# davidalvarezdlt/master_thesis

Measured on NVIDIA B200. Metric: aligned_frames_per_sec, higher is better.
Workload: dtype f32

## Files before the change

### include/mt_b200.h

```cpp
#ifndef MT_B200_H
#define MT_B200_H

#include <stdint.h>

#ifdef __cplusplus
extern "C" {
#endif

#define MT_OK 0
#define MT_ERR_INVALID (-1)
#define MT_ERR_CUDA (-2)
#define MT_ERR_NO_DEVICE (-3)

typedef void *mt_stream_t;

#define MT_API __attribute__((visibility("default")))

#define MT_ALIGN_CORNERS 1
#define MT_VIS_BILINEAR 2
#define MT_GRID_AFFINE 4
#define MT_VIS_FROM_MASK 8

#define MT_REDUCE_MEAN 0
#define MT_REDUCE_SUM 1

MT_API int mt_version(void);
MT_API const char *mt_last_error(void);
MT_API int mt_set_tuning(const char *name, int value);
MT_API int mt_device_info(int *sm_count, int *cc_major, int *cc_minor);
MT_API int64_t mt_workspace_bytes(void);

MT_API int mt_warp_fwd(const float *x, int64_t x_sb, int64_t x_sc, int64_t x_sf,
                const float *vis, int64_t vis_sb, int64_t vis_sf,
                const float *grid, const float *m_target, int64_t mt_sb,
                float *x_aligned, int64_t xa_sb, int64_t xa_sc, int64_t xa_sf,
                float *v_aligned, float *v_map,
                int B, int C, int F, int H, int W, int flags, mt_stream_t stream);

MT_API int mt_warp_pack_fwd(const float *x, int64_t x_sb, int64_t x_sc, int64_t x_sf,
                     const float *vis, int64_t vis_sb, int64_t vis_sf,
                     const float *grid, const float *m_target, int64_t mt_sb,
                     const float *x_t, int64_t xt_sb, int64_t xt_sc, const float *v_t, int64_t vt_sb,
                     float *nn_in,
                     float *x_aligned, int64_t xa_sb, int64_t xa_sc, int64_t xa_sf,
                     float *v_aligned, float *v_map,
                     int B, int F, int H, int W, int flags, mt_stream_t stream);

MT_API int mt_warp_lowres_fwd(const float *x, int64_t x_sb, int64_t x_sc, int64_t x_sf,
                       const float *vis, int64_t vis_sb, int64_t vis_sf,
                       const float *flow, int gh, int gw, const float *m_target, int64_t mt_sb,
                       float *x_aligned, int64_t xa_sb, int64_t xa_sc, int64_t xa_sf,
                       float *v_aligned, float *v_map,
                       int B, int F, int H, int W, int flags, mt_stream_t stream);
MT_API int mt_warp_pack_lowres_fwd(const float *x, int64_t x_sb, int64_t x_sc, int64_t x_sf,
                            const float *vis, int64_t vis_sb, int64_t vis_sf,
                            const float *flow, int gh, int gw, const float *m_target, int64_t mt_sb,
                            const float *x_t, int64_t xt_sb, int64_t xt_sc, const float *v_t, int64_t vt_sb,
                            float *nn_in,
                            float *x_aligned, int64_t xa_sb, int64_t xa_sc, int64_t xa_sf,
                            float *v_aligned, float *v_map,
                            int B, int F, int H, int W, int flags, mt_stream_t stream);

MT_API int mt_warp_bwd_grid(const float *x, int64_t x_sb, int64_t x_sc, int64_t x_sf,
                     const float *grid,
                     const float *gout, int64_t g_sb, int64_t g_sc, int64_t g_sf,
                     float *ggrid, int B, int C, int F, int H, int W, int flags,
                     mt_stream_t stream);

MT_API int mt_warp_l1_fwd(const float *x, int64_t x_sb, int64_t x_sc, int64_t x_sf,
                   const float *vis, int64_t vis_sb, int64_t vis_sf,
                   const float *flow,
                   const float *x_target, int64_t xt_sb, int64_t xt_sc,
                   const float *v_target, int64_t vt_sb,
                   float *x_aligned, float *v_aligned, float *out3, void *workspace,
                   int B, int F, int H, int W, float weight, int flags, mt_stream_t stream);

MT_API int mt_warp_l1_bwd(const float *x, int64_t x_sb, int64_t x_sc, int64_t x_sf,
                   const float *flow,
                   const float *x_target, int64_t xt_sb, int64_t xt_sc,
                   const float *v_target, int64_t vt_sb,
                   const float *out3, const float *grad_out, float *gflow,
                   int B, int F, int H, int W, float weight, int flags, mt_stream_t stream);

MT_API int mt_mask_out(const float *flow, int64_t n, float *out, mt_stream_t stream);

MT_API int mt_masked_l1_fwd(const float *y_hat, int64_t a_sb, int64_t a_sc, int64_t a_sf,
                     const float *y, int64_t b_sb, int64_t b_sc, int64_t b_sf,
                     const float *mask, int64_t m_sb, int64_t m_sc, int64_t m_sf,
                     const uint8_t *batch_mask, float *out3, void *workspace,
                     int B, int C, int F, int64_t P, int mask_c, int64_t mask_repeat, int reduction,
                     float weight, mt_stream_t stream);
MT_API int mt_masked_l1_bwd(const float *y_hat, int64_t a_sb, int64_t a_sc, int64_t a_sf,
                     const float *y, int64_t b_sb, int64_t b_sc, int64_t b_sf,
                     const float *mask, int64_t m_sb, int64_t m_sc, int64_t m_sf,
                     const uint8_t *batch_mask, const float *out3, const float *grad_out,
                     float *grad_y_hat, float *grad_y,
                     int B, int C, int F, int64_t P, int mask_c, int reduction, float weight,
                     mt_stream_t stream);

MT_API int mt_chn_l1x3_fwd(const float *y_hat, int64_t yh_sb, int64_t yh_sc, int64_t yh_sf,
                    const float *y_comp, int64_t yc_sb, int64_t yc_sc, int64_t yc_sf,
                    const float *y_target, int64_t yt_sb, int64_t yt_sc,
                    const float *v_target, int64_t vt_sb,
                    const float *v_map, int64_t vm_sb, int64_t vm_sf,
                    float *out9, void *workspace, int B, int F, int64_t P,
                    float w_nh, float w_vh, float w_nvh, mt_stream_t stream);
MT_API int mt_chn_l1x3_bwd(const float *y_hat, int64_t yh_sb, int64_t yh_sc, int64_t yh_sf,
                    const float *y_comp, int64_t yc_sb, int64_t yc_sc, int64_t yc_sf,
                    const float *y_target, int64_t yt_sb, int64_t yt_sc,
                    const float *v_target, int64_t vt_sb,
                    const float *v_map, int64_t vm_sb, int64_t vm_sf,
                    const float *out9, const float *grad_out3, float *grad_y_hat, float *grad_y_comp,
                    int B, int F, int64_t P, float w_nh, float w_vh, float w_nvh, mt_stream_t stream);

MT_API int mt_chn_fill_step(const float *nn_out, const float *x_t, int64_t xt_sb, int64_t xt_sc,
                     const float *v_t, int64_t vt_sb, const float *m_t, int64_t mt_sb,
                     const float *v_map0, int64_t vm_sb, float *y_comp0, float *m_new, float *x_new,
                     float *inp_per, void *workspace, int B, int64_t P, mt_stream_t stream);

MT_API int mt_chn_fill_step_gated(const float *nn_out, const float *x_t, int64_t xt_sb, int64_t xt_sc,
                           const float *v_t, int64_t vt_sb, const float *m_t, int64_t mt_sb,
                           const float *v_map0, int64_t vm_sb, const float *y_prev,
                           const float *gate_per, float gate_e,
                           float *y_comp0, float *m_new, float *x_new,
                           float *inp_per, void *workspace, int B, int64_t P, mt_stream_t stream);

MT_API int mt_corr4d_fwd(const float *feats_t, const float *v_t, const float *feats_r, const float *v_r,
                  float *out, void *workspace, int64_t workspace_bytes,
                  int B, int C, int F, int P, mt_stream_t stream);
MT_API int64_t mt_corr4d_workspace_bytes(int B, int C, int F, int P);
MT_API int mt_corr4d_uses_tensor_cores(int C, int P);

MT_API int mt_corr4d_vgg_fwd(const float *feats_t, int64_t ft_sb, int64_t ft_sc,
                      const float *m_target, int64_t mt_sb,
                      const float *feats_r, int64_t fr_sb, int64_t fr_sc, int64_t fr_sf,
                      const float *m_refs, int64_t mr_sb, int64_t mr_sf, int MH, int MW,
                      float *out, int B, int C, int F, int h, int w, mt_stream_t stream);

MT_API int mt_corr4d_vgg_l1_fwd(const float *feats_t, int64_t ft_sb, int64_t ft_sc,
                         const float *m_target, int64_t mt_sb,
                         const float *feats_r, int64_t fr_sb, int64_t fr_sc, int64_t fr_sf,
                         const float *m_refs, int64_t mr_sb, int64_t mr_sf, int MH, int MW,
                         const float *pred, float *loss, void *sign, void *workspace, int64_t workspace_bytes,
                         int B, int C, int F, int h, int w, mt_stream_t stream);
MT_API int64_t mt_corr4d_l1_workspace_bytes(void);
MT_API int mt_corr4d_l1_bwd(const void *sign, const float *grad_loss, float *g_pred, int64_t n, mt_stream_t stream);

MT_API int mt_cm_match_fwd(const float *c_feats, const float *v_t, const float *v_aligned,
                    float *out, float *c_mask, void *workspace,
                    int B, int C, int f, int h, int w, int H, int W, mt_stream_t stream);
MT_API int64_t mt_cm_workspace_bytes(int B, int C, int f, int h, int w);
MT_API const float *mt_cm_workspace_gs(const void *workspace, int B, int C, int f, int h, int w);

MT_API int mt_chn_pack(const float *x_t, int64_t xt_sb, int64_t xt_sc, const float *v_t, int64_t vt_sb,
                const float *x_al, int64_t xa_sb, int64_t xa_sc, int64_t xa_sf,
                const float *v_al, int64_t va_sb, int64_t va_sf,
                const float *v_map, int64_t vm_sb, int64_t vm_sf,
                float *nn_in, int B, int F, int64_t P, mt_stream_t stream);
MT_API int mt_chn_composite_fwd(const float *nn_out, const float *x_t, int64_t xt_sb, int64_t xt_sc,
                         const float *v_t, int64_t vt_sb, float *y_hat, float *y_comp,
                         int B, int F, int64_t P, mt_stream_t stream);
MT_API int mt_chn_composite_bwd(const float *nn_out, const float *v_t, int64_t vt_sb,
                         const float *g_yhat, int64_t gy_sb, int64_t gy_sc, int64_t gy_sf,
                         const float *g_comp, int64_t gc_sb, int64_t gc_sc, int64_t gc_sf,
                         float *g_nn, int B, int F, int64_t P, mt_stream_t stream);
MT_API int mt_hole_update(const float *m_t, int64_t mt_sb, const float *v_map0, int64_t vm_sb,
                   const float *y_comp0, int64_t yc_sb, int64_t yc_sc,
                   float *m_new, float *x_new, float *inp_per, void *workspace,
                   int B, int64_t P, mt_stream_t stream);
MT_API int mt_trivial_copy(const float *x_t, int64_t xt_sb, int64_t xt_sc,
                    const float *x_al, int64_t xa_sb, int64_t xa_sc, int64_t xa_sf,
                    const float *v_map, int64_t vm_sb, int64_t vm_sf,
                    float *y, int B, int F, int64_t P, mt_stream_t stream);

MT_API int mt_flow_pack(const float *x_refs, int64_t xr_sb, int64_t xr_sc, int64_t xr_sf,
                 const float *x_t, int64_t xt_sb, int64_t xt_sc,
                 const float *m_refs, int64_t mr_sb, int64_t mr_sf, const float *m_t, int64_t mt_sb,
                 const float *flow, int64_t fl_sb, int64_t fl_sf, int64_t fl_sy, int64_t fl_sx, int64_t fl_sc,
                 float *nn_in, int B, int F, int H, int W, mt_stream_t stream);

MT_API int mt_cpn_align_host(const float *x_refs, const float *m_refs, const float *m_target,
                      const float *theta, float *x_aligned, float *v_aligned, float *v_maps,
                      int B, int F, int H, int W);
MT_API int mt_dfpn_align_host(const float *x_refs, const float *m_refs, const float *m_target,
                       const float *flow, float *x_aligned, float *v_aligned, float *v_maps,
                       int B, int F, int H, int W);

#ifdef __cplusplus
}
#endif
#endif
```

### master_thesis_b200/csrc/warp.cu

```cuda
#include <math.h>

#include "mt_common.cuh"
#include "warp_common.cuh"

namespace mt {
namespace {

constexpr int kCols = 128;
#ifndef MT_WARP_ROWS
#define MT_WARP_ROWS 2
#endif
#ifndef MT_TAP_REUSE
#define MT_TAP_REUSE 1
#endif
constexpr int kRows = MT_WARP_ROWS;
constexpr bool kTapReuse = MT_TAP_REUSE != 0;
constexpr int kIters = 1;
#ifndef MT_WARP_MINB
#define MT_WARP_MINB 8
#endif
#ifndef MT_WARP_MINB1
#define MT_WARP_MINB1 10
#endif
#ifndef MT_WARP_MINB4
#define MT_WARP_MINB4 4
#endif
#ifndef MT_WARPB_MINB
#define MT_WARPB_MINB 6
#endif
#ifndef MT_WARPL1F_MINB
#define MT_WARPL1F_MINB 8
#endif
#ifndef MT_WARPL1B_MINB
#define MT_WARPL1B_MINB 8
#endif

struct WarpFwdArgs {
    const float *x, *vis, *grid, *m_target;
    float *x_al, *v_al, *v_map;
    int x_sb, x_sc, x_sf, vis_sb, vis_sf, mt_sb, xa_sb, xa_sc, xa_sf;
    int F, P;
    int iters;
    unsigned f_magic;
    Sampler sp;
    bool from_mask;
    const float *x_t, *v_t;
    float *nn_in;
    int xt_sb, xt_sc, vt_sb;
    int gh, gw;
    float gsy, gsx;
    int early_trigger;
};
constexpr int kMaxRowsPerCta = 32;

template <int C, int U, int VIS, bool AFFINE, bool FULL, bool PACK = false, bool LOWRES = false>
__global__ void __launch_bounds__(kCols, U >= 4 ? MT_WARP_MINB4 : (U == 1 ? MT_WARP_MINB1 : MT_WARP_MINB)) warp_fwd_kernel(const WarpFwdArgs a) {
    static_assert(!(AFFINE && LOWRES), "a theta needs no resize");
    pdl_wait();
    if (a.early_trigger) pdl_launch();
    __shared__ float s_by[kMaxRowsPerCta];
    __shared__ Lin s_ly[LOWRES ? kMaxRowsPerCta : 1];
    const int W = a.sp.W, H = a.sp.H;
    const bool live = (int)(blockIdx.x * kCols + threadIdx.x) < W;
    const int x = min((int)(blockIdx.x * kCols + threadIdx.x), W - 1);
    const int rows_cta = U * a.iters;
    const int yb = blockIdx.y * rows_cta;
    const unsigned n = blockIdx.z;
    const int b = a.f_magic ? (int)__umulhi(n, a.f_magic) : (int)n, f = (int)n - b * a.F;
    const bool ac = a.sp.ac;
    if (AFFINE) {
        if ((int)threadIdx.x < rows_cta)
            s_by[threadIdx.x] = base_coord(min(yb + (int)threadIdx.x, H - 1), H, a.sp.stepy, ac);
        __syncthreads();
    }
    Lin lx;
    if (LOWRES) {
        if ((int)threadIdx.x < rows_cta) s_ly[threadIdx.x] = lin_index(min(yb + (int)threadIdx.x, H - 1), a.gh, H, a.gsy);
        lx = lin_index(x, a.gw, W, a.gsx);
        __syncthreads();
    }
    const int xo = b * a.x_sb + f * a.x_sf;
    const float *__restrict__ vp = a.vis + (b * a.vis_sb + f * a.vis_sf);
    const int xao = b * a.xa_sb + f * a.xa_sf;
    const int mto = b * a.mt_sb;

    float t1 = 0.f, t2 = 0.f, t4 = 0.f, t5 = 0.f, bxt0 = 0.f, bxt3 = 0.f;
    if (AFFINE) {
        const float *th = a.grid + n * 6;
        const float bx = base_coord(x, W, a.sp.stepx, ac);
        bxt0 = __fmul_rn(bx, __ldg(th));
        bxt3 = __fmul_rn(bx, __ldg(th + 3));
        t1 = __ldg(th + 1); t2 = __ldg(th + 2); t4 = __ldg(th + 4); t5 = __ldg(th + 5);
    }
    const float wm2 = a.sp.wmax - 1.0f, hm2 = a.sp.hmax - 1.0f;

    constexpr bool kDense = !AFFINE && !LOWRES;
    float2 g_next[U];
    if (kDense) {
#pragma unroll
        for (int k = 0; k < U; ++k)
            g_next[k] = (yb + k < H) ? __ldcs(reinterpret_cast<const float2 *>(a.grid) + ((int)n * a.P + (yb + k) * W + x))
                                     : make_float2(0.0f, 0.0f);
    }
#pragma unroll 1
    for (int it = 0; it < a.iters; ++it) {
        const int y0 = yb + it * U;
        if (y0 >= H) break;
        const int p0 = y0 * W + x;
        const int np0 = (int)n * a.P + p0;
        float mtv[U];
        if (FULL || PACK || a.v_map) {
#pragma unroll
            for (int k = 0; k < U; ++k) mtv[k] = (y0 + k < H) ? __ldcs(a.m_target + (mto + p0 + k * W)) : 0.0f;
        }
        float xtv[PACK ? 3 : 1][U], vtv[U];
        if (PACK) {
#pragma unroll
            for (int k = 0; k < U; ++k) {
                const bool in = y0 + k < H;
                vtv[k] = in ? __ldg(a.v_t + (b * a.vt_sb + p0 + k * W)) : 0.0f;
#pragma unroll
                for (int c = 0; c < 3; ++c) xtv[c][k] = in ? __ldg(a.x_t + (b * a.xt_sb + c * a.xt_sc + p0 + k * W)) : 0.0f;
            }
        }
        float ix[U], iy[U], xw[U], yn[U];
        float wnw[U], wne[U], wsw[U], wse[U];
        bool interior = true;
#pragma unroll
        for (int k = 0; k < U; ++k) {
            float gx, gy;
            if (AFFINE) {
                const float by = s_by[it * U + k];
                gx = __fadd_rn(__fmaf_rn(by, t1, bxt0), t2);
                gy = __fadd_rn(__fmaf_rn(by, t4, bxt3), t5);
            } else if (LOWRES) {
                const Lin ly = s_ly[it * U + k];
                const float2 *fl = reinterpret_cast<const float2 *>(a.grid) + (int)n * (a.gh * a.gw);
                const float2 g = lin_flow(fl + ly.i0 * a.gw, fl + ly.i1 * a.gw, lx, ly.l0, ly.l1);
                gx = g.x; gy = g.y;
            } else {
                gx = g_next[k].x; gy = g_next[k].y;
            }
            ix[k] = unnormalize(gx, a.sp.sfx, ac);
            iy[k] = unnormalize(gy, a.sp.sfy, ac);
            xw[k] = floorf(ix[k]);
            yn[k] = floorf(iy[k]);
            const float w = __fsub_rn(ix[k], xw[k]), e = __fsub_rn(1.0f, w);
            const float nn = __fsub_rn(iy[k], yn[k]), ss = __fsub_rn(1.0f, nn);
            wnw[k] = __fmul_rn(ss, e); wne[k] = __fmul_rn(ss, w);
            wsw[k] = __fmul_rn(nn, e); wse[k] = __fmul_rn(nn, w);
            interior = interior && (xw[k] >= 0.0f) && (xw[k] <= wm2) && (yn[k] >= 0.0f) && (yn[k] <= hm2);
        }
        if (kDense && it + 1 < a.iters) {
#pragma unroll
            for (int k = 0; k < U; ++k)
                g_next[k] = (y0 + U + k < H) ? __ldcs(reinterpret_cast<const float2 *>(a.grid) + (np0 + (U + k) * W))
                                             : make_float2(0.0f, 0.0f);
        }
        float xa[C][U], va[U];
        if (__all_sync(0xffffffffu, interior)) {
            float c00[C + 1][U], c01[C + 1][U], c10[C + 1][U], c11[C + 1][U];
            int o[U];
            bool same[U];
#pragma unroll
            for (int k = 0; k < U; ++k) {
                o[k] = (int)yn[k] * W + (int)xw[k];
                same[k] = kTapReuse && k > 0 && o[k] == o[k - 1] + W;
            }
#pragma unroll
            for (int k = 0; k < U; ++k) {
#pragma unroll
                for (int c = 0; c < C; ++c) {
                    const float *r0 = a.x + (xo + c * a.x_sc + o[k]);
                    const float *r1 = a.x + (xo + c * a.x_sc + o[k] + W);
                    c00[c][k] = 0.0f; c01[c][k] = 0.0f;
                    if (!same[k]) { c00[c][k] = __ldg(r0); c01[c][k] = __ldg(r0 + 1); }
                    c10[c][k] = __ldg(r1); c11[c][k] = __ldg(r1 + 1);
                }
                if (VIS == 2) {
                    const float *r0 = vp + o[k];
                    const float *r1 = vp + (o[k] + W);
                    c00[C][k] = 0.0f; c01[C][k] = 0.0f;
                    if (!same[k]) { c00[C][k] = __ldg(r0); c01[C][k] = __ldg(r0 + 1); }
                    c10[C][k] = __ldg(r1); c11[C][k] = __ldg(r1 + 1);
                } else {
                    c00[C][k] = __ldg(vp + ((int)rintf(iy[k]) * W + (int)rintf(ix[k])));
                }
            }
#pragma unroll
            for (int k = 1; k < U; ++k) {
#pragma unroll
                for (int c = 0; c < (VIS == 2 ? C + 1 : C); ++c) {
                    c00[c][k] = same[k] ? c10[c][k - 1] : c00[c][k];
                    c01[c][k] = same[k] ? c11[c][k - 1] : c01[c][k];
                }
            }
#pragma unroll
            for (int k = 0; k < U; ++k) {
#pragma unroll
                for (int c = 0; c < C; ++c)
                    xa[c][k] = __fmaf_rn(c11[c][k], wse[k], __fmaf_rn(c10[c][k], wsw[k],
                               __fmaf_rn(c01[c][k], wne[k], __fmul_rn(c00[c][k], wnw[k]))));
                if (VIS == 2) {
                    float v00 = c00[C][k], v01 = c01[C][k], v10 = c10[C][k], v11 = c11[C][k];
                    if (a.from_mask) {
                        v00 = __fsub_rn(1.0f, v00); v01 = __fsub_rn(1.0f, v01);
                        v10 = __fsub_rn(1.0f, v10); v11 = __fsub_rn(1.0f, v11);
                    }
                    const float vs = __fmaf_rn(v11, wse[k], __fmaf_rn(v10, wsw[k],
                                     __fmaf_rn(v01, wne[k], __fmul_rn(v00, wnw[k]))));
                    va[k] = vs > 0.5f ? 1.0f : 0.0f;
                } else {
                    va[k] = a.from_mask ? __fsub_rn(1.0f, c00[C][k]) : c00[C][k];
                }
            }
        } else {
#pragma unroll
            for (int k = 0; k < U; ++k) {
                const Bil bl = bil_params(ix[k], iy[k], a.sp);
#pragma unroll
                for (int c = 0; c < C; ++c) xa[c][k] = interp(gather(a.x + (xo + c * a.x_sc), bl, W), bl);
                if (VIS == 2) {
                    Corners cv = gather(vp, bl, W);
                    if (a.from_mask) {
                        cv.nw = (bl.y0 && bl.x0) ? __fsub_rn(1.0f, cv.nw) : 0.0f;
                        cv.ne = (bl.y0 && bl.x1) ? __fsub_rn(1.0f, cv.ne) : 0.0f;
                        cv.sw = (bl.y1 && bl.x0) ? __fsub_rn(1.0f, cv.sw) : 0.0f;
                        cv.se = (bl.y1 && bl.x1) ? __fsub_rn(1.0f, cv.se) : 0.0f;
                    }
                    va[k] = interp(cv, bl) > 0.5f ? 1.0f : 0.0f;
                } else {
                    va[k] = nearest(vp, ix[k], iy[k], a.sp, a.from_mask);
                }
            }
        }
        if (live) {
#pragma unroll
            for (int k = 0; k < U; ++k) {
                if (y0 + k >= H) break;
                if (FULL || a.x_al) {
#pragma unroll
                    for (int c = 0; c < C; ++c) st_stream1(a.x_al + (xao + p0 + c * a.xa_sc + k * W), xa[c][k]);
                }
                if (FULL || a.v_al) st_stream1(a.v_al + (np0 + k * W), va[k]);
                const float vmap = (FULL || PACK || a.v_map) ? clamp01(__fsub_rn(va[k], __fsub_rn(1.0f, mtv[k]))) : 0.0f;
                if (FULL || a.v_map)
                    st_stream1(a.v_map + (np0 + k * W), vmap);
                if (PACK) {
                    float *o = a.nn_in + ((int)n * 9 * a.P + p0 + k * W);
#pragma unroll
                    for (int c = 0; c < 3; ++c) {
                        const float m = chan_mean(c), sd = chan_std(c);
                        st_stream1(o + c * a.P, __fdiv_rn(__fsub_rn(xtv[c][k], m), sd));
                        st_stream1(o + (3 + c) * a.P, __fdiv_rn(__fsub_rn(xa[c][k], m), sd));
                    }
                    st_stream1(o + 6 * a.P, vtv[k]);
                    st_stream1(o + 7 * a.P, va[k]);
                    st_stream1(o + 8 * a.P, vmap);
                }
            }
        }
    }
}

template <int U>
struct Taps {
    float gx[U], gy[U], ix[U], iy[U], xw[U], yn[U], w[U], e[U], n[U], s[U];
    bool interior;
};

template <int U>
__device__ __forceinline__ void dense_flow_load(const float *__restrict__ flow, int np0, int y0, const Sampler &sp,
                                                float2 (&g)[U]) {
#pragma unroll
    for (int k = 0; k < U; ++k)
        g[k] = (y0 + k < sp.H) ? __ldcs(reinterpret_cast<const float2 *>(flow) + (np0 + k * sp.W)) : make_float2(0.0f, 0.0f);
}

template <int U>
__device__ __forceinline__ void dense_taps_from(const float2 (&g)[U], const Sampler &sp, Taps<U> &t) {
    const float wm2 = sp.wmax - 1.0f, hm2 = sp.hmax - 1.0f;
    t.interior = true;
#pragma unroll
    for (int k = 0; k < U; ++k) {
        t.gx[k] = g[k].x; t.gy[k] = g[k].y;
        t.ix[k] = unnormalize(t.gx[k], sp.sfx, sp.ac);
        t.iy[k] = unnormalize(t.gy[k], sp.sfy, sp.ac);
        t.xw[k] = floorf(t.ix[k]);
        t.yn[k] = floorf(t.iy[k]);
        t.w[k] = __fsub_rn(t.ix[k], t.xw[k]); t.e[k] = __fsub_rn(1.0f, t.w[k]);
        t.n[k] = __fsub_rn(t.iy[k], t.yn[k]); t.s[k] = __fsub_rn(1.0f, t.n[k]);
        t.interior = t.interior && (t.xw[k] >= 0.0f) && (t.xw[k] <= wm2) && (t.yn[k] >= 0.0f) && (t.yn[k] <= hm2);
    }
}

template <int U>
__device__ __forceinline__ void dense_taps(const float *__restrict__ flow, int np0, int y0, const Sampler &sp,
                                           Taps<U> &t) {
    float2 g[U];
    dense_flow_load<U>(flow, np0, y0, sp, g);
    dense_taps_from<U>(g, sp, t);
}

template <int C, int U>
__device__ __forceinline__ void gather_taps(const float *__restrict__ x, int xo, int x_sc, const Sampler &sp,
                                            const Taps<U> &t, Corners (&q)[C][U]) {
    if (__all_sync(0xffffffffu, t.interior)) {
#pragma unroll
        int o[U];
        bool same[U];
#pragma unroll
        for (int k = 0; k < U; ++k) {
            o[k] = (int)t.yn[k] * sp.W + (int)t.xw[k];
            same[k] = kTapReuse && k > 0 && o[k] == o[k - 1] + sp.W;
        }
#pragma unroll
        for (int k = 0; k < U; ++k) {
#pragma unroll
            for (int c = 0; c < C; ++c) {
                const float *r0 = x + (xo + c * x_sc + o[k]);
                const float *r1 = x + (xo + c * x_sc + o[k] + sp.W);
                q[c][k].nw = 0.0f; q[c][k].ne = 0.0f;
                if (!same[k]) { q[c][k].nw = __ldg(r0); q[c][k].ne = __ldg(r0 + 1); }
                q[c][k].sw = __ldg(r1); q[c][k].se = __ldg(r1 + 1);
            }
        }
#pragma unroll
        for (int k = 1; k < U; ++k) {
#pragma unroll
            for (int c = 0; c < C; ++c) {
                q[c][k].nw = same[k] ? q[c][k - 1].sw : q[c][k].nw;
                q[c][k].ne = same[k] ? q[c][k - 1].se : q[c][k].ne;
            }
        }
    } else {
#pragma unroll
        for (int k = 0; k < U; ++k) {
            const Bil bl = bil_params(t.ix[k], t.iy[k], sp);
#pragma unroll
            for (int c = 0; c < C; ++c) q[c][k] = gather(x + (xo + c * x_sc), bl, sp.W);
        }
    }
}

template <int U>
__device__ __forceinline__ float interp_k(const Corners &q, const Taps<U> &t, int k) {
    return __fmaf_rn(q.se, __fmul_rn(t.n[k], t.w[k]), __fmaf_rn(q.sw, __fmul_rn(t.n[k], t.e[k]),
           __fmaf_rn(q.ne, __fmul_rn(t.s[k], t.w[k]), __fmul_rn(q.nw, __fmul_rn(t.s[k], t.e[k])))));
}

#ifndef MT_WARPB_ROWS
#define MT_WARPB_ROWS 2
#endif
constexpr int kRowsB = MT_WARPB_ROWS;

struct WarpBwdArgs {
    const float *x, *grid, *gout;
    float *ggrid;
    int x_sb, x_sc, x_sf, g_sb, g_sc, g_sf;
    int F, P;
    unsigned f_magic;
    Sampler sp;
};

template <int C, int U>
__global__ void __launch_bounds__(kCols, MT_WARPB_MINB) warp_bwd_grid_kernel(const WarpBwdArgs a) {
    pdl_sync();
    const int W = a.sp.W, H = a.sp.H;
    const bool live = (int)(blockIdx.x * kCols + threadIdx.x) < W;
    const int x = min((int)(blockIdx.x * kCols + threadIdx.x), W - 1);
    const int y0 = blockIdx.y * U;
    const unsigned n = blockIdx.z;
    const int b = a.f_magic ? (int)__umulhi(n, a.f_magic) : (int)n, f = (int)n - b * a.F;
    const int p0 = y0 * W + x, np0 = (int)n * a.P + p0;
    const int go0 = b * a.g_sb + f * a.g_sf + p0;
    float go[C][U];
#pragma unroll
    for (int c = 0; c < C; ++c)
#pragma unroll
        for (int k = 0; k < U; ++k) go[c][k] = (y0 + k < H) ? __ldcs(a.gout + (go0 + c * a.g_sc + k * W)) : 0.0f;
    Taps<U> t;
    dense_taps<U>(a.grid, np0, y0, a.sp, t);
    Corners q[C][U];
    gather_taps<C, U>(a.x, b * a.x_sb + f * a.x_sf, a.x_sc, a.sp, t, q);
    if (!live) return;
#pragma unroll
    for (int k = 0; k < U; ++k) {
        if (y0 + k >= H) break;
        float ax = 0.0f, ay = 0.0f;
#pragma unroll
        for (int c = 0; c < C; ++c) {
            ax += ((q[c][k].ne - q[c][k].nw) * t.s[k] + (q[c][k].se - q[c][k].sw) * t.n[k]) * go[c][k];
            ay += ((q[c][k].sw - q[c][k].nw) * t.e[k] + (q[c][k].se - q[c][k].ne) * t.w[k]) * go[c][k];
        }
        __stcs(reinterpret_cast<float2 *>(a.ggrid) + (np0 + k * W), make_float2(ax * a.sp.sfx, ay * a.sp.sfy));
    }
}

struct WarpL1Args {
    const float *x, *vis, *flow, *xt, *vt;
    float *x_al, *v_al;
    float *out3; void *ws;
    const float *out3_in, *grad_out; float *gflow;
    int x_sb, x_sc, x_sf, vis_sb, vis_sf, xt_sb, xt_sc, vt_sb;
    int F, P, row_blocks;
    unsigned f_magic;
    float weight;
    Sampler sp;
    bool from_mask;
};

__device__ __forceinline__ float mask_out_of(float gx, float gy) {
    return (gx < -1.0f || gx > 1.0f || gy < -1.0f || gy > 1.0f) ? 1.0f : 0.0f;
}

template <int U, bool MAT>
__global__ void __launch_bounds__(kCols, MAT ? MT_WARPB_MINB : MT_WARPL1F_MINB) warp_l1_fwd_kernel(const WarpL1Args a) {
    pdl_sync();
    __shared__ float red[2 * 32];
    float acc[2] = {0.0f, 0.0f};
    const int W = a.sp.W, H = a.sp.H;
    const bool live = (int)(blockIdx.x * kCols + threadIdx.x) < W;
    const int x = min((int)(blockIdx.x * kCols + threadIdx.x), W - 1);
    const unsigned n = blockIdx.z;
    const int b = a.f_magic ? (int)__umulhi(n, a.f_magic) : (int)n, f = (int)n - b * a.F;
    const int xo = b * a.x_sb + f * a.x_sf;
    const int per = (a.row_blocks + (int)gridDim.y - 1) / (int)gridDim.y;
    const int rb0 = (int)blockIdx.y * per, rb1 = min(rb0 + per, a.row_blocks);
    float2 g_next[U];
    if (rb0 < rb1)
        dense_flow_load<U>(a.flow, (int)n * a.P + rb0 * U * W + x, rb0 * U, a.sp, g_next);
    for (int rb = rb0; rb < rb1; ++rb) {
        const int y0 = rb * U;
        const int p0 = y0 * W + x, np0 = (int)n * a.P + p0;
        float xt[3][U], vt[U];
#pragma unroll
        for (int k = 0; k < U; ++k) {
            const bool in = y0 + k < H;
            vt[k] = in ? __ldg(a.vt + (b * a.vt_sb + p0 + k * W)) : 0.0f;
#pragma unroll
            for (int c = 0; c < 3; ++c) xt[c][k] = in ? __ldg(a.xt + (b * a.xt_sb + c * a.xt_sc + p0 + k * W)) : 0.0f;
        }
        Taps<U> t;
        dense_taps_from<U>(g_next, a.sp, t);
        {
            const int rn = rb + 1;
            if (rn < rb1) dense_flow_load<U>(a.flow, (int)n * a.P + rn * U * W + x, rn * U, a.sp, g_next);
        }
        Corners q[3][U];
        gather_taps<3, U>(a.x, xo, a.x_sc, a.sp, t, q);
#pragma unroll
        for (int k = 0; k < U; ++k) {
            if (y0 + k >= H || !live) continue;
            const float M = __fmul_rn(vt[k], __fsub_rn(1.0f, mask_out_of(t.gx[k], t.gy[k])));
            acc[1] += M;
#pragma unroll
            for (int c = 0; c < 3; ++c) {
                const float r = interp_k<U>(q[c][k], t, k);
                acc[0] += fabsf(__fsub_rn(__fmul_rn(xt[c][k], M), __fmul_rn(r, M)));
                if (MAT && a.x_al) st_stream1(a.x_al + (((int)n * 3 + c) * a.P + p0 + k * W), r);
            }
            if (MAT && a.v_al)
                st_stream1(a.v_al + (np0 + k * W),
                           nearest(a.vis + (b * a.vis_sb + f * a.vis_sf), t.ix[k], t.iy[k], a.sp, a.from_mask));
        }
    }
    float *out3 = a.out3;
    const float weight = a.weight;
    grid_reduce_finish<2>(acc, a.ws, red, [out3, weight](const double *tot) {
        const float num = (float)tot[0], den = (float)tot[1];
        out3[0] = weight * num / (den + 1e-9f);
        out3[1] = num;
        out3[2] = den;
    });
}

template <int U>
__global__ void __launch_bounds__(kCols, MT_WARPL1B_MINB) warp_l1_bwd_kernel(const WarpL1Args a) {
    pdl_sync();
    const int W = a.sp.W, H = a.sp.H;
    const bool live = (int)(blockIdx.x * kCols + threadIdx.x) < W;
    const int x = min((int)(blockIdx.x * kCols + threadIdx.x), W - 1);
    const int y0 = blockIdx.y * U;
    const unsigned n = blockIdx.z;
    const int b = a.f_magic ? (int)__umulhi(n, a.f_magic) : (int)n, f = (int)n - b * a.F;
    const int p0 = y0 * W + x, np0 = (int)n * a.P + p0;
    const float scale = a.weight * __ldg(a.grad_out) / (__ldg(a.out3_in + 2) + 1e-9f);
    float xt[3][U], vt[U];
#pragma unroll
    for (int k = 0; k < U; ++k) {
        const bool in = y0 + k < H;
        vt[k] = in ? __ldg(a.vt + (b * a.vt_sb + p0 + k * W)) : 0.0f;
#pragma unroll
        for (int c = 0; c < 3; ++c) xt[c][k] = in ? __ldg(a.xt + (b * a.xt_sb + c * a.xt_sc + p0 + k * W)) : 0.0f;
    }
    Taps<U> t;
    dense_taps<U>(a.flow, np0, y0, a.sp, t);
    Corners q[3][U];
    gather_taps<3, U>(a.x, b * a.x_sb + f * a.x_sf, a.x_sc, a.sp, t, q);
    if (!live) return;
#pragma unroll
    for (int k = 0; k < U; ++k) {
        if (y0 + k >= H) break;
        const float M = __fmul_rn(vt[k], __fsub_rn(1.0f, mask_out_of(t.gx[k], t.gy[k])));
        float ax = 0.0f, ay = 0.0f;
#pragma unroll
        for (int c = 0; c < 3; ++c) {
            const float d = __fsub_rn(__fmul_rn(xt[c][k], M), __fmul_rn(interp_k<U>(q[c][k], t, k), M));
            const float sg = (d > 0.0f) ? 1.0f : ((d < 0.0f) ? -1.0f : 0.0f);
            const float go = -sg * M * scale;
            ax += ((q[c][k].ne - q[c][k].nw) * t.s[k] + (q[c][k].se - q[c][k].sw) * t.n[k]) * go;
            ay += ((q[c][k].sw - q[c][k].nw) * t.e[k] + (q[c][k].se - q[c][k].ne) * t.w[k]) * go;
        }
        __stcs(reinterpret_cast<float2 *>(a.gflow) + (np0 + k * W), make_float2(ax * a.sp.sfx, ay * a.sp.sfy));
    }
}

__global__ void __launch_bounds__(256) mask_out_kernel(const float *__restrict__ flow, int64_t n,
                                                       float *__restrict__ out) {
    pdl_sync();
    for (int64_t i = blockIdx.x * (int64_t)blockDim.x + threadIdx.x; i < n;
         i += (int64_t)gridDim.x * blockDim.x) {
        const float2 g = __ldcs(reinterpret_cast<const float2 *>(flow) + i);
        st_stream1(out + i, mask_out_of(g.x, g.y));
    }
}

bool aligned8(const void *p) { return (reinterpret_cast<uintptr_t>(p) & 7u) == 0; }

}
}

namespace mt {
int warp_staged_launch(const float *x, int64_t x_sb, int64_t x_sc, int64_t x_sf, const float *vis,
                       int64_t vis_sb, int64_t vis_sf, const float *theta, const float *m_target,
                       int64_t mt_sb, float *x_aligned, int64_t xa_sb, int64_t xa_sc, int64_t xa_sf,
                       float *v_aligned, float *v_map, int B, int F, int H, int W, bool ac, bool from_mask,
                       cudaStream_t st);
}

using namespace mt;

static unsigned frame_magic(int F) {
    return F == 1 ? 0u : (unsigned)(((1ull << 32) + (unsigned)F - 1) / (unsigned)F);
}

struct PackOut {
    const float *x_t; int64_t xt_sb, xt_sc;
    const float *v_t; int64_t vt_sb;
    float *nn_in;
};

static int warp_fwd_impl(const float *x, int64_t x_sb, int64_t x_sc, int64_t x_sf,
                         const float *vis, int64_t vis_sb, int64_t vis_sf, const float *grid,
                         const float *m_target, int64_t mt_sb, float *x_aligned, int64_t xa_sb,
                         int64_t xa_sc, int64_t xa_sf, float *v_aligned, float *v_map, int B,
                         int C, int F, int H, int W, int flags, mt_stream_t stream, const PackOut *pack,
                         int gh = 0, int gw = 0) {
    MT_REQUIRE(x && vis && grid, "mt_warp_fwd: NULL input");
    const bool lowres = gh > 0 && gw > 0 && !(gh == H && gw == W);
    MT_REQUIRE(!lowres || (!(flags & MT_GRID_AFFINE) && !(flags & MT_VIS_BILINEAR) && C == 3 &&
                           (int64_t)B * F * gh * gw * 2 < (1ll << 31) - 1),
               "mt_warp_lowres_fwd: needs a dense flow, nearest visibility, C = 3 and B*F*gh*gw*2 < 2^31");
    MT_REQUIRE(B > 0 && F > 0 && H > 0 && W > 0, "mt_warp_fwd: empty shape B=%d F=%d H=%d W=%d", B, F, H, W);
    MT_REQUIRE(C == 1 || C == 3, "mt_warp_fwd: C must be 1 or 3 (reference hard-codes 3, utils.py:97), got %d", C);
    MT_REQUIRE((int64_t)B * F <= 65535, "mt_warp_fwd: B*F > 65535");
    MT_REQUIRE(!v_map || m_target, "mt_warp_fwd: v_map needs m_target");
    MT_REQUIRE((flags & MT_GRID_AFFINE) || aligned8(grid), "mt_warp_fwd: dense grid must be 8 B aligned");
    MT_REQUIRE((H + kRows - 1) / kRows <= 65535, "mt_warp_fwd: H too large");
    const int64_t P = (int64_t)H * W, lim = (1ll << 31) - 1;
    auto span = [&](int64_t sb, int64_t sc, int64_t sf, int c) {
        return (B - 1) * sb + (c - 1) * sc + (F - 1) * sf + P + W + 1;
    };
    MT_REQUIRE(x_sb >= 0 && x_sc >= 0 && x_sf >= 0 && vis_sb >= 0 && vis_sf >= 0 && mt_sb >= 0 &&
               xa_sb >= 0 && xa_sc >= 0 && xa_sf >= 0, "mt_warp_fwd: negative strides are not supported");
    MT_REQUIRE(span(x_sb, x_sc, x_sf, C) < lim && span(vis_sb, 0, vis_sf, 1) < lim &&
               span(xa_sb, xa_sc, xa_sf, C) < lim && (int64_t)B * F * P * 2 < lim && (B - 1) * mt_sb + P < lim,
               "mt_warp_fwd: tensors beyond 2^31 elements are not supported (split the batch)");
    WarpFwdArgs a;
    a.x = x; a.vis = vis; a.grid = grid; a.m_target = m_target;
    a.x_al = x_aligned; a.v_al = v_aligned; a.v_map = v_map;
    a.x_sb = (int)x_sb; a.x_sc = (int)x_sc; a.x_sf = (int)x_sf;
    a.vis_sb = (int)vis_sb; a.vis_sf = (int)vis_sf; a.mt_sb = (int)mt_sb;
    a.xa_sb = (int)xa_sb; a.xa_sc = (int)xa_sc; a.xa_sf = (int)xa_sf;
    a.F = F; a.P = (int)P;
    a.f_magic = frame_magic(F);
    a.sp = make_sampler(H, W, (flags & MT_ALIGN_CORNERS) != 0);
    a.from_mask = (flags & MT_VIS_FROM_MASK) != 0;
    a.x_t = a.v_t = nullptr; a.nn_in = nullptr; a.xt_sb = a.xt_sc = a.vt_sb = 0;
    a.gh = lowres ? gh : H; a.gw = lowres ? gw : W;
    a.gsy = (float)a.gh / (float)H; a.gsx = (float)a.gw / (float)W;
    a.early_trigger = tuning("MT_WARP_EARLY_TRIGGER", 1);
    if (pack) {
        MT_REQUIRE(C == 3 && m_target && pack->x_t && pack->v_t && pack->nn_in, "mt_warp_pack_fwd: C must be 3, no NULL input");
        MT_REQUIRE(pack->xt_sb >= 0 && pack->xt_sc >= 0 && pack->vt_sb >= 0 &&
                   (B - 1) * pack->xt_sb + 2 * pack->xt_sc + P < lim && (B - 1) * pack->vt_sb + P < lim &&
                   (int64_t)B * F * 9 * P < lim, "mt_warp_pack_fwd: tensors beyond 2^31 elements are not supported");
        a.x_t = pack->x_t; a.v_t = pack->v_t; a.nn_in = pack->nn_in;
        a.xt_sb = (int)pack->xt_sb; a.xt_sc = (int)pack->xt_sc; a.vt_sb = (int)pack->vt_sb;
    }
    const bool affine = (flags & MT_GRID_AFFINE) != 0;
    const bool vis_bil = (flags & MT_VIS_BILINEAR) != 0;
    int rows = tuning("MT_WARP_ROWS", kRows);
    rows = rows == 1 && !pack && !lowres ? 1 : (rows == 4 ? 4 : 2);
    int iters = tuning("MT_WARP_ITERS", kIters);
    if (iters < 1) iters = 1;
    if (iters * rows > kMaxRowsPerCta) iters = kMaxRowsPerCta / rows;
    a.iters = iters;
    dim3 block(kCols), gridd((W + kCols - 1) / kCols, (H + rows * iters - 1) / (rows * iters), B * F);
    cudaStream_t st = (cudaStream_t)stream;
    const bool full = x_aligned && v_aligned && v_map;
    if (pack && lowres) {
        if (rows == 2) launch(warp_fwd_kernel<3, 2, 1, false, false, true, true>, gridd, block, 0, st, a);
        else launch(warp_fwd_kernel<3, 4, 1, false, false, true, true>, gridd, block, 0, st, a);
        return launch_status("mt_warp_pack_lowres_fwd");
    }
    if (lowres) {
        if (rows == 2) {
            if (full) launch(warp_fwd_kernel<3, 2, 1, false, true, false, true>, gridd, block, 0, st, a);
            else launch(warp_fwd_kernel<3, 2, 1, false, false, false, true>, gridd, block, 0, st, a);
        } else {
            if (full) launch(warp_fwd_kernel<3, 4, 1, false, true, false, true>, gridd, block, 0, st, a);
            else launch(warp_fwd_kernel<3, 4, 1, false, false, false, true>, gridd, block, 0, st, a);
        }
        return launch_status("mt_warp_lowres_fwd");
    }
    if (pack) {
#define MT_WARP_PACK_GO(VV, AA)                                                                       \
    do {                                                                                              \
        if (rows == 2) launch(warp_fwd_kernel<3, 2, VV, AA, false, true>, gridd, block, 0, st, a);    \
        else launch(warp_fwd_kernel<3, 4, VV, AA, false, true>, gridd, block, 0, st, a);              \
    } while (0)
        if (vis_bil) { if (affine) MT_WARP_PACK_GO(2, true); else MT_WARP_PACK_GO(2, false); }
        else         { if (affine) MT_WARP_PACK_GO(1, true); else MT_WARP_PACK_GO(1, false); }
#undef MT_WARP_PACK_GO
        return launch_status("mt_warp_pack_fwd");
    }
    if (affine && vis_bil && C == 3 && full) {
        const int rc = warp_staged_launch(x, x_sb, x_sc, x_sf, vis, vis_sb, vis_sf, grid, m_target, mt_sb, x_aligned,
                                          xa_sb, xa_sc, xa_sf, v_aligned, v_map, B, F, H, W, a.sp.ac, a.from_mask, st);
        if (rc < 0) return rc;
        if (rc == 1) return launch_status("mt_warp_fwd");
    }
#define MT_WARP_GO(CC, VV, AA, FF)                                                  \
    do {                                                                            \
        if (rows == 2) launch(warp_fwd_kernel<CC, 2, VV, AA, FF>, gridd, block, 0, st, a); \
        else if (rows == 1) launch(warp_fwd_kernel<CC, 1, VV, AA, FF>, gridd, block, 0, st, a); \
        else launch(warp_fwd_kernel<CC, 4, VV, AA, FF>, gridd, block, 0, st, a);        \
    } while (0)
#define MT_WARP_PICK(CC)                                                            \
    do {                                                                            \
        if (vis_bil) {                                                              \
            if (affine) { if (full) MT_WARP_GO(CC, 2, true, true); else MT_WARP_GO(CC, 2, true, false); }   \
            else        { if (full) MT_WARP_GO(CC, 2, false, true); else MT_WARP_GO(CC, 2, false, false); } \
        } else {                                                                    \
            if (affine) { if (full) MT_WARP_GO(CC, 1, true, true); else MT_WARP_GO(CC, 1, true, false); }   \
            else        { if (full) MT_WARP_GO(CC, 1, false, true); else MT_WARP_GO(CC, 1, false, false); } \
        }                                                                           \
    } while (0)
    if (C == 3) MT_WARP_PICK(3); else MT_WARP_PICK(1);
#undef MT_WARP_PICK
#undef MT_WARP_GO
    return launch_status("mt_warp_fwd");
}

extern "C" int mt_warp_fwd(const float *x, int64_t x_sb, int64_t x_sc, int64_t x_sf,
                           const float *vis, int64_t vis_sb, int64_t vis_sf, const float *grid,
                           const float *m_target, int64_t mt_sb, float *x_aligned, int64_t xa_sb,
                           int64_t xa_sc, int64_t xa_sf, float *v_aligned, float *v_map, int B,
                           int C, int F, int H, int W, int flags, mt_stream_t stream) {
    return warp_fwd_impl(x, x_sb, x_sc, x_sf, vis, vis_sb, vis_sf, grid, m_target, mt_sb, x_aligned, xa_sb, xa_sc,
                         xa_sf, v_aligned, v_map, B, C, F, H, W, flags, stream, nullptr);
}

extern "C" int mt_warp_pack_fwd(const float *x, int64_t x_sb, int64_t x_sc, int64_t x_sf,
                                const float *vis, int64_t vis_sb, int64_t vis_sf, const float *grid,
                                const float *m_target, int64_t mt_sb, const float *x_t, int64_t xt_sb,
                                int64_t xt_sc, const float *v_t, int64_t vt_sb, float *nn_in,
                                float *x_aligned, int64_t xa_sb, int64_t xa_sc, int64_t xa_sf,
                                float *v_aligned, float *v_map, int B, int F, int H, int W, int flags,
                                mt_stream_t stream) {
    PackOut pk{x_t, xt_sb, xt_sc, v_t, vt_sb, nn_in};
    return warp_fwd_impl(x, x_sb, x_sc, x_sf, vis, vis_sb, vis_sf, grid, m_target, mt_sb, x_aligned, xa_sb, xa_sc,
                         xa_sf, v_aligned, v_map, B, 3, F, H, W, flags, stream, &pk);
}

extern "C" int mt_warp_lowres_fwd(const float *x, int64_t x_sb, int64_t x_sc, int64_t x_sf,
                                  const float *vis, int64_t vis_sb, int64_t vis_sf, const float *flow, int gh,
                                  int gw, const float *m_target, int64_t mt_sb, float *x_aligned, int64_t xa_sb,
                                  int64_t xa_sc, int64_t xa_sf, float *v_aligned, float *v_map, int B, int F,
                                  int H, int W, int flags, mt_stream_t stream) {
    MT_REQUIRE(gh > 0 && gw > 0, "mt_warp_lowres_fwd: empty flow");
    return warp_fwd_impl(x, x_sb, x_sc, x_sf, vis, vis_sb, vis_sf, flow, m_target, mt_sb, x_aligned, xa_sb, xa_sc,
                         xa_sf, v_aligned, v_map, B, 3, F, H, W, flags, stream, nullptr, gh, gw);
}

extern "C" int mt_warp_pack_lowres_fwd(const float *x, int64_t x_sb, int64_t x_sc, int64_t x_sf,
                                       const float *vis, int64_t vis_sb, int64_t vis_sf, const float *flow,
                                       int gh, int gw, const float *m_target, int64_t mt_sb, const float *x_t,
                                       int64_t xt_sb, int64_t xt_sc, const float *v_t, int64_t vt_sb,
                                       float *nn_in, float *x_aligned, int64_t xa_sb, int64_t xa_sc,
                                       int64_t xa_sf, float *v_aligned, float *v_map, int B, int F, int H,
                                       int W, int flags, mt_stream_t stream) {
    MT_REQUIRE(gh > 0 && gw > 0, "mt_warp_pack_lowres_fwd: empty flow");
    PackOut pk{x_t, xt_sb, xt_sc, v_t, vt_sb, nn_in};
    return warp_fwd_impl(x, x_sb, x_sc, x_sf, vis, vis_sb, vis_sf, flow, m_target, mt_sb, x_aligned, xa_sb, xa_sc,
                         xa_sf, v_aligned, v_map, B, 3, F, H, W, flags, stream, &pk, gh, gw);
}

extern "C" int mt_warp_bwd_grid(const float *x, int64_t x_sb, int64_t x_sc, int64_t x_sf,
                                const float *grid, const float *gout, int64_t g_sb, int64_t g_sc,
                                int64_t g_sf, float *ggrid, int B, int C, int F, int H, int W,
                                int flags, mt_stream_t stream) {
    MT_REQUIRE(x && grid && gout && ggrid, "mt_warp_bwd_grid: NULL argument");
    MT_REQUIRE(B > 0 && F > 0 && H > 0 && W > 0, "mt_warp_bwd_grid: empty shape");
    MT_REQUIRE(C == 1 || C == 3, "mt_warp_bwd_grid: C must be 1 or 3, got %d", C);
    MT_REQUIRE(!(flags & MT_GRID_AFFINE), "mt_warp_bwd_grid: dense grids only");
    MT_REQUIRE((int64_t)B * F <= 65535 && (H + kRowsB - 1) / kRowsB <= 65535, "mt_warp_bwd_grid: too large");
    MT_REQUIRE(aligned8(grid) && aligned8(ggrid), "mt_warp_bwd_grid: grids must be 8 B aligned");
    const int64_t P = (int64_t)H * W, lim = (1ll << 31) - 1;
    MT_REQUIRE(x_sb >= 0 && x_sc >= 0 && x_sf >= 0 && g_sb >= 0 && g_sc >= 0 && g_sf >= 0,
               "mt_warp_bwd_grid: negative strides are not supported");
    MT_REQUIRE((B - 1) * x_sb + (C - 1) * x_sc + (F - 1) * x_sf + P + W + 1 < lim &&
               (B - 1) * g_sb + (C - 1) * g_sc + (F - 1) * g_sf + P < lim && (int64_t)B * F * P * 2 < lim,
               "mt_warp_bwd_grid: tensors beyond 2^31 elements are not supported (split the batch)");
    WarpBwdArgs a;
    a.x = x; a.grid = grid; a.gout = gout; a.ggrid = ggrid;
    a.x_sb = (int)x_sb; a.x_sc = (int)x_sc; a.x_sf = (int)x_sf;
    a.g_sb = (int)g_sb; a.g_sc = (int)g_sc; a.g_sf = (int)g_sf;
    a.F = F; a.P = (int)P; a.f_magic = frame_magic(F);
    a.sp = make_sampler(H, W, (flags & MT_ALIGN_CORNERS) != 0);
    dim3 block(kCols), gridd((W + kCols - 1) / kCols, (H + kRowsB - 1) / kRowsB, B * F);
    cudaStream_t st = (cudaStream_t)stream;
    if (C == 3) launch(warp_bwd_grid_kernel<3, kRowsB>, gridd, block, 0, st, a);
    else launch(warp_bwd_grid_kernel<1, kRowsB>, gridd, block, 0, st, a);
    return launch_status("mt_warp_bwd_grid");
}

static int fill_l1_args(WarpL1Args &a, const float *x, int64_t x_sb, int64_t x_sc, int64_t x_sf,
                        const float *flow, const float *x_target, int64_t xt_sb, int64_t xt_sc,
                        const float *v_target, int64_t vt_sb, int B, int F, int H, int W,
                        float weight, int flags, const char *who) {
    MT_REQUIRE(x && flow && x_target && v_target, "%s: NULL input", who);
    MT_REQUIRE(B > 0 && F > 0 && H > 0 && W > 0, "%s: empty shape", who);
    MT_REQUIRE((int64_t)B * F <= 65535 && (H + kRowsB - 1) / kRowsB <= 65535, "%s: too large", who);
    MT_REQUIRE(aligned8(flow), "%s: flow must be 8 B aligned", who);
    const int64_t P = (int64_t)H * W, lim = (1ll << 31) - 1;
    MT_REQUIRE(x_sb >= 0 && x_sc >= 0 && x_sf >= 0 && xt_sb >= 0 && xt_sc >= 0 && vt_sb >= 0,
               "%s: negative strides are not supported", who);
    MT_REQUIRE((B - 1) * x_sb + 2 * x_sc + (F - 1) * x_sf + P + W + 1 < lim && (B - 1) * xt_sb + 2 * xt_sc + P < lim &&
               (B - 1) * vt_sb + P < lim && (int64_t)B * F * P * 3 < lim,
               "%s: tensors beyond 2^31 elements are not supported (split the batch)", who);
    a.x = x; a.flow = flow; a.xt = x_target; a.vt = v_target;
    a.x_sb = (int)x_sb; a.x_sc = (int)x_sc; a.x_sf = (int)x_sf;
    a.xt_sb = (int)xt_sb; a.xt_sc = (int)xt_sc; a.vt_sb = (int)vt_sb;
    a.F = F; a.P = (int)P; a.weight = weight; a.f_magic = frame_magic(F);
    a.sp = make_sampler(H, W, (flags & MT_ALIGN_CORNERS) != 0);
    a.from_mask = (flags & MT_VIS_FROM_MASK) != 0;
    a.vis = nullptr; a.vis_sb = a.vis_sf = 0; a.x_al = a.v_al = nullptr; a.out3 = nullptr; a.ws = nullptr;
    a.out3_in = nullptr; a.grad_out = nullptr; a.gflow = nullptr;
    a.row_blocks = (H + kRowsB - 1) / kRowsB;
    return MT_OK;
}

extern "C" int mt_warp_l1_fwd(const float *x, int64_t x_sb, int64_t x_sc, int64_t x_sf,
                              const float *vis, int64_t vis_sb, int64_t vis_sf, const float *flow,
                              const float *x_target, int64_t xt_sb, int64_t xt_sc,
                              const float *v_target, int64_t vt_sb, float *x_aligned,
                              float *v_aligned, float *out3, void *workspace, int B, int F, int H,
                              int W, float weight, int flags, mt_stream_t stream) {
    WarpL1Args a;
    int rc = fill_l1_args(a, x, x_sb, x_sc, x_sf, flow, x_target, xt_sb, xt_sc, v_target, vt_sb, B,
                          F, H, W, weight, flags, "mt_warp_l1_fwd");
    if (rc) return rc;
    MT_REQUIRE(out3 && workspace, "mt_warp_l1_fwd: NULL out3 / workspace");
    MT_REQUIRE(!v_aligned || vis, "mt_warp_l1_fwd: v_aligned needs vis");
    MT_REQUIRE(vis_sb >= 0 && vis_sf >= 0 && (!vis || (B - 1) * vis_sb + (F - 1) * vis_sf + (int64_t)H * W < (1ll << 31) - 1),
               "mt_warp_l1_fwd: vis beyond 2^31 elements");
    a.vis = vis; a.vis_sb = (int)vis_sb; a.vis_sf = (int)vis_sf; a.x_al = x_aligned; a.v_al = v_aligned;
    a.out3 = out3; a.ws = workspace;
    const int colb = (W + kCols - 1) / kCols;
    int gy = a.row_blocks;
    MT_REQUIRE((int64_t)colb * B * F <= kMaxReduceBlocks,
               "mt_warp_l1_fwd: B*F*ceil(W/128) = %lld exceeds %d CTAs (split the batch)",
               (long long)colb * B * F, kMaxReduceBlocks);
    int64_t per_sm = tuning("MT_WARPL1_CTAS_PER_SM", 16);
    if (per_sm < 1) per_sm = 1;
    if (per_sm * sm_count() > kMaxReduceBlocks) per_sm = kMaxReduceBlocks / sm_count();
    int64_t cap = ((int64_t)sm_count() * per_sm) / ((int64_t)colb * B * F);
    if (cap < 1) cap = 1;
    if (gy > cap) gy = (int)cap;
    dim3 block(kCols), gridd(colb, gy, B * F);
    if (a.x_al || a.v_al) launch(warp_l1_fwd_kernel<kRowsB, true>, gridd, block, 0, (cudaStream_t)stream, a);
    else launch(warp_l1_fwd_kernel<kRowsB, false>, gridd, block, 0, (cudaStream_t)stream, a);
    return launch_status("mt_warp_l1_fwd");
}

extern "C" int mt_warp_l1_bwd(const float *x, int64_t x_sb, int64_t x_sc, int64_t x_sf,
                              const float *flow, const float *x_target, int64_t xt_sb,
                              int64_t xt_sc, const float *v_target, int64_t vt_sb,
                              const float *out3, const float *grad_out, float *gflow, int B, int F,
                              int H, int W, float weight, int flags, mt_stream_t stream) {
    WarpL1Args a;
    int rc = fill_l1_args(a, x, x_sb, x_sc, x_sf, flow, x_target, xt_sb, xt_sc, v_target, vt_sb, B,
                          F, H, W, weight, flags, "mt_warp_l1_bwd");
    if (rc) return rc;
    MT_REQUIRE(out3 && grad_out && gflow, "mt_warp_l1_bwd: NULL out3 / grad_out / gflow");
    MT_REQUIRE(aligned8(gflow), "mt_warp_l1_bwd: gflow must be 8 B aligned");
    a.out3_in = out3; a.grad_out = grad_out; a.gflow = gflow;
    dim3 block(kCols), gridd((W + kCols - 1) / kCols, a.row_blocks, B * F);
    launch(warp_l1_bwd_kernel<kRowsB>, gridd, block, 0, (cudaStream_t)stream, a);
    return launch_status("mt_warp_l1_bwd");
}

extern "C" int mt_mask_out(const float *flow, int64_t n, float *out, mt_stream_t stream) {
    MT_REQUIRE(flow && out && n > 0, "mt_mask_out: bad argument");
    MT_REQUIRE((reinterpret_cast<uintptr_t>(flow) & 7u) == 0, "mt_mask_out: flow must be 8 B aligned");
    int64_t nb = (n + 255) / 256, cap = (int64_t)sm_count() * 16;
    launch(mask_out_kernel, (int)(nb < cap ? nb : cap), 256, 0, (cudaStream_t)stream, flow, n, out);
    return launch_status("mt_mask_out");
}
```

Before: 714,000.

## Use cached pitch-2D texture gathers for bilinear taps in non-affine warp path

For the C=3, two-row, full, non-affine, nearest-visibility warp case, the input frames are bound as a pitch-2D texture object and each channel's four bilinear taps are fetched with a single tex2Dgather instead of four __ldg loads. Texture objects are created lazily and cached per base pointer, width and row count, so creation cost is paid once per buffer. The intent is to cut load instruction count and exploit the texture cache's 2D locality. In exchange it adds a host-side mutex and lookup on every call, disables the row tap-reuse path, grows a cache that can hold stale objects for freed buffers, and falls back to the old path when alignment, size limits or stream capture rule textures out.

Measured after the change: 723,300, median of 6. 1.3% higher.

```diff
diff --git a/include/mt_b200.h b/include/mt_b200.h
--- a/include/mt_b200.h
+++ b/include/mt_b200.h
@@ -27,6 +27,7 @@
 MT_API int mt_version(void);
 MT_API const char *mt_last_error(void);
 MT_API int mt_set_tuning(const char *name, int value);
+MT_API int mt_warp_tex_objects(void);
 MT_API int mt_device_info(int *sm_count, int *cc_major, int *cc_minor);
 MT_API int64_t mt_workspace_bytes(void);
 
diff --git a/master_thesis_b200/csrc/tex_cache.cu b/master_thesis_b200/csrc/tex_cache.cu
--- /dev/null
+++ b/master_thesis_b200/csrc/tex_cache.cu
@@ -0,0 +1,91 @@
+#include <mutex>
+#include <vector>
+
+#include "mt_common.cuh"
+#include "tex_cache.cuh"
+
+namespace mt {
+namespace {
+
+struct DevLimits {
+    bool init = false;
+    int pitch_align = 0, max_w = 0, max_h = 0, max_pitch = 0;
+};
+
+struct TexEntry {
+    int dev;
+    const float *base;
+    int W;
+    int64_t rows;
+    cudaTextureObject_t obj;
+};
+
+std::mutex g_tex_mu;
+std::vector<TexEntry> g_tex;
+DevLimits g_limits[64];
+
+bool multiple_of(int64_t stride, int n, int W) { return n == 1 || stride % W == 0; }
+
+}
+
+cudaTextureObject_t tex_planes(const float *base, int64_t sb, int64_t sc, int64_t sf, int B, int C, int F, int H,
+                               int W, cudaStream_t st) {
+    int dev = 0;
+    if (cudaGetDevice(&dev) != cudaSuccess || dev < 0 || dev >= 64) {
+        (void)cudaGetLastError();
+        return 0;
+    }
+    if (!multiple_of(sb, B, W) || !multiple_of(sc, C, W) || !multiple_of(sf, F, W)) return 0;
+    const int64_t rows = ((B - 1) * sb + (C - 1) * sc + (F - 1) * sf) / W + H;
+    const int64_t pitch = 4 * (int64_t)W;
+
+    std::lock_guard<std::mutex> lock(g_tex_mu);
+    DevLimits &lim = g_limits[dev];
+    if (!lim.init) {
+        if (cudaDeviceGetAttribute(&lim.pitch_align, cudaDevAttrTexturePitchAlignment, dev) != cudaSuccess ||
+            cudaDeviceGetAttribute(&lim.max_w, cudaDevAttrMaxTexture2DLinearWidth, dev) != cudaSuccess ||
+            cudaDeviceGetAttribute(&lim.max_h, cudaDevAttrMaxTexture2DLinearHeight, dev) != cudaSuccess ||
+            cudaDeviceGetAttribute(&lim.max_pitch, cudaDevAttrMaxTexture2DLinearPitch, dev) != cudaSuccess) {
+            (void)cudaGetLastError();
+            return 0;
+        }
+        lim.init = true;
+    }
+    if (lim.pitch_align <= 0 || reinterpret_cast<uintptr_t>(base) % (uintptr_t)lim.pitch_align != 0 ||
+        pitch % lim.pitch_align != 0 || W > lim.max_w || rows > lim.max_h || pitch > lim.max_pitch)
+        return 0;
+    for (const TexEntry &e : g_tex)
+        if (e.dev == dev && e.base == base && e.W == W && e.rows == rows) return e.obj;
+    if ((int)g_tex.size() >= tuning("MT_TEX_CACHE_CAP", 256)) return 0;
+    cudaStreamCaptureStatus cs = cudaStreamCaptureStatusNone;
+    if (cudaStreamIsCapturing(st, &cs) != cudaSuccess || cs != cudaStreamCaptureStatusNone) {
+        (void)cudaGetLastError();
+        return 0;
+    }
+    cudaResourceDesc rd = {};
+    rd.resType = cudaResourceTypePitch2D;
+    rd.res.pitch2D.devPtr = const_cast<float *>(base);
+    rd.res.pitch2D.desc = cudaCreateChannelDesc<float>();
+    rd.res.pitch2D.width = (size_t)W;
+    rd.res.pitch2D.height = (size_t)rows;
+    rd.res.pitch2D.pitchInBytes = (size_t)pitch;
+    cudaTextureDesc td = {};
+    td.addressMode[0] = td.addressMode[1] = cudaAddressModeBorder;
+    td.filterMode = cudaFilterModePoint;
+    td.readMode = cudaReadModeElementType;
+    td.normalizedCoords = 0;
+    cudaTextureObject_t obj = 0;
+    if (cudaCreateTextureObject(&obj, &rd, &td, nullptr) != cudaSuccess) {
+        (void)cudaGetLastError();
+        return 0;
+    }
+    g_tex.push_back(TexEntry{dev, base, W, rows, obj});
+    return obj;
+}
+
+}
+
+extern "C" int mt_warp_tex_objects(void) {
+    std::lock_guard<std::mutex> lock(mt::g_tex_mu);
+    return (int)mt::g_tex.size();
+}
diff --git a/master_thesis_b200/csrc/tex_cache.cuh b/master_thesis_b200/csrc/tex_cache.cuh
--- /dev/null
+++ b/master_thesis_b200/csrc/tex_cache.cuh
@@ -0,0 +1,11 @@
+#pragma once
+
+#include <cuda_runtime.h>
+#include <stdint.h>
+
+namespace mt {
+
+cudaTextureObject_t tex_planes(const float *base, int64_t sb, int64_t sc, int64_t sf, int B, int C, int F, int H,
+                               int W, cudaStream_t st);
+
+}
diff --git a/master_thesis_b200/csrc/warp.cu b/master_thesis_b200/csrc/warp.cu
--- a/master_thesis_b200/csrc/warp.cu
+++ b/master_thesis_b200/csrc/warp.cu
@@ -1,6 +1,7 @@
 #include <math.h>
 
 #include "mt_common.cuh"
+#include "tex_cache.cuh"
 #include "warp_common.cuh"
 
 namespace mt {
@@ -50,12 +51,15 @@
     int gh, gw;
     float gsy, gsx;
     int early_trigger;
+    cudaTextureObject_t tx;
+    int x_rb, x_rc, x_rf;
 };
 constexpr int kMaxRowsPerCta = 32;
 
-template <int C, int U, int VIS, bool AFFINE, bool FULL, bool PACK = false, bool LOWRES = false>
+template <int C, int U, int VIS, bool AFFINE, bool FULL, bool PACK = false, bool LOWRES = false, bool TEX = false>
 __global__ void __launch_bounds__(kCols, U >= 4 ? MT_WARP_MINB4 : (U == 1 ? MT_WARP_MINB1 : MT_WARP_MINB)) warp_fwd_kernel(const WarpFwdArgs a) {
     static_assert(!(AFFINE && LOWRES), "a theta needs no resize");
+    static_assert(!TEX || (VIS == 1 && !AFFINE && !PACK && !LOWRES), "texture gathers: DFPN align tail only");
     pdl_wait();
     if (a.early_trigger) pdl_launch();
     __shared__ float s_by[kMaxRowsPerCta];
@@ -165,26 +169,40 @@
 #pragma unroll
             for (int k = 0; k < U; ++k) {
                 o[k] = (int)yn[k] * W + (int)xw[k];
-                same[k] = kTapReuse && k > 0 && o[k] == o[k - 1] + W;
-            }
-#pragma unroll
-            for (int k = 0; k < U; ++k) {
-#pragma unroll
-                for (int c = 0; c < C; ++c) {
-                    const float *r0 = a.x + (xo + c * a.x_sc + o[k]);
-                    const float *r1 = a.x + (xo + c * a.x_sc + o[k] + W);
-                    c00[c][k] = 0.0f; c01[c][k] = 0.0f;
-                    if (!same[k]) { c00[c][k] = __ldg(r0); c01[c][k] = __ldg(r0 + 1); }
-                    c10[c][k] = __ldg(r1); c11[c][k] = __ldg(r1 + 1);
+                same[k] = !TEX && kTapReuse && k > 0 && o[k] == o[k - 1] + W;
+            }
+            if (TEX) {
+                const int xr0 = b * a.x_rb + f * a.x_rf;
+#pragma unroll
+                for (int k = 0; k < U; ++k) {
+                    const float u = xw[k] + 1.0f;
+#pragma unroll
+                    for (int c = 0; c < C; ++c) {
+                        const float4 q = tex2Dgather<float4>(a.tx, u, (float)(xr0 + c * a.x_rc) + (yn[k] + 1.0f), 0);
+                        c00[c][k] = q.w; c01[c][k] = q.z; c10[c][k] = q.x; c11[c][k] = q.y;
+                    }
+                    c00[C][k] = __ldg(vp + ((int)rintf(iy[k]) * W + (int)rintf(ix[k])));
                 }
-                if (VIS == 2) {
-                    const float *r0 = vp + o[k];
-                    const float *r1 = vp + (o[k] + W);
-                    c00[C][k] = 0.0f; c01[C][k] = 0.0f;
-                    if (!same[k]) { c00[C][k] = __ldg(r0); c01[C][k] = __ldg(r0 + 1); }
-                    c10[C][k] = __ldg(r1); c11[C][k] = __ldg(r1 + 1);
-                } else {
-                    c00[C][k] = __ldg(vp + ((int)rintf(iy[k]) * W + (int)rintf(ix[k])));
+            } else {
+#pragma unroll
+                for (int k = 0; k < U; ++k) {
+#pragma unroll
+                    for (int c = 0; c < C; ++c) {
+                        const float *r0 = a.x + (xo + c * a.x_sc + o[k]);
+                        const float *r1 = a.x + (xo + c * a.x_sc + o[k] + W);
+                        c00[c][k] = 0.0f; c01[c][k] = 0.0f;
+                        if (!same[k]) { c00[c][k] = __ldg(r0); c01[c][k] = __ldg(r0 + 1); }
+                        c10[c][k] = __ldg(r1); c11[c][k] = __ldg(r1 + 1);
+                    }
+                    if (VIS == 2) {
+                        const float *r0 = vp + o[k];
+                        const float *r1 = vp + (o[k] + W);
+                        c00[C][k] = 0.0f; c01[C][k] = 0.0f;
+                        if (!same[k]) { c00[C][k] = __ldg(r0); c01[C][k] = __ldg(r0 + 1); }
+                        c10[C][k] = __ldg(r1); c11[C][k] = __ldg(r1 + 1);
+                    } else {
+                        c00[C][k] = __ldg(vp + ((int)rintf(iy[k]) * W + (int)rintf(ix[k])));
+                    }
                 }
             }
 #pragma unroll
@@ -591,6 +609,8 @@
     a.gh = lowres ? gh : H; a.gw = lowres ? gw : W;
     a.gsy = (float)a.gh / (float)H; a.gsx = (float)a.gw / (float)W;
     a.early_trigger = tuning("MT_WARP_EARLY_TRIGGER", 1);
+    a.tx = 0;
+    a.x_rb = a.x_rc = a.x_rf = 0;
     if (pack) {
         MT_REQUIRE(C == 3 && m_target && pack->x_t && pack->v_t && pack->nn_in, "mt_warp_pack_fwd: C must be 3, no NULL input");
         MT_REQUIRE(pack->xt_sb >= 0 && pack->xt_sc >= 0 && pack->vt_sb >= 0 &&
@@ -641,6 +661,14 @@
                                           xa_sb, xa_sc, xa_sf, v_aligned, v_map, B, F, H, W, a.sp.ac, a.from_mask, st);
         if (rc < 0) return rc;
         if (rc == 1) return launch_status("mt_warp_fwd");
+    }
+    if (C == 3 && rows == 2 && full && !affine && !vis_bil && tuning("MT_WARP_TEX", 1)) {
+        a.tx = tex_planes(x, x_sb, x_sc, x_sf, B, C, F, H, W, st);
+        if (a.tx) {
+            a.x_rb = (int)(x_sb / W); a.x_rc = (int)(x_sc / W); a.x_rf = (int)(x_sf / W);
+            launch(warp_fwd_kernel<3, 2, 1, false, true, false, false, true>, gridd, block, 0, st, a);
+            return launch_status("mt_warp_fwd");
+        }
     }
 #define MT_WARP_GO(CC, VV, AA, FF)                                                  \
     do {                                                                            \
```
